# chlhnu/DOT-SOCP

Measured on AMD Instinct MI355X. Metric: ADMM iters/sec on NxNxT dot2d staggered grid at 1/2/4/8 MI355X, higher is better.
Workload: dtype f64

## Files before the change

### dot-socp_amd/csrc/kernels.h

```cpp
#pragma once
#include "common.h"
#include "defer.h"
#include "particle_block.h"

namespace dotsocp {

struct LoopCoef {
    double s;
    double sf;
    double dF;
    double at, ax, ay;
    double tau;
    double c1, c2;
    double dinv1, dinv2;
};

enum {
    S_Q2 = 0, S_Z2, S_APHI2, S_ALPHA2, S_BETA2, S_FBBETA2, S_PRIM1, S_PRIM2, S_DUAL1, S_DUAL2,
    S_COMPLEM, S_DOTCOMP, S_RHO2, S_RHOFQ2, S_MRHOB, S_M2, S_RHOB2, S_QALPHA, S_CPHI, S_PHI2,
    S_COUNT
};

struct KktCoef {
    double sigma;
// ... 134 lines not shown
#define HL_XCHUNK_MAX 32
int launch_hl_pass_y(bool forward, const double *in, double *out, int *arg, i64 n, i64 lines, i64 pitch, hipStream_t st);
int launch_hl_pass_x(bool forward, const double *in, double *out, int *arg, i64 n, i64 lines, i64 pitch, hipStream_t st);
int hl_chunk(int deflt);
int launch_hl_layer(const double *in, double *out, i64 n, double mul, hipStream_t st);
enum { HS_M0 = 0, HS_M1, HS_P0R0, HS_P1R1, HS_HR1, HS_BR0, HS_G1, HS_G0, HS_MAP, HS_COUNT };
enum { HC_G1_MAX = 0, HC_G1_MIN, HC_G0_MAX, HC_G0_MIN, HC_NONFINITE, HC_COUNT };
struct HlReduceArgs {
    i64 ny, nx, py;
    const double *phi0, *phi1, *H, *B, *rho0, *rho1;
    const int *ixf, *iyf, *ixb, *iyb;
    int *arg_fwd, *arg_bwd;
    double hx, hy;
    double *partials;
    unsigned long long *counts;
};
i64 hl_blocks(i64 nodes);
int launch_hl_reduce(const HlReduceArgs &a, double *sums , hipStream_t st);

enum { RR_MAX = 0, RR_MIN, RR_NONFINITE, RR_MASKED, RR_COUNT };
#define RND_LEVELS 255
int launch_rho_range(const Grid &g, const double *alpha, const double *weight, const double *rho0, const double *rho1,
                     const double *a_prev, double sig, double cD, const unsigned char *barrier, unsigned long long *counts,
                     hipStream_t st);
int launch_render(const Grid &g, const double *alpha, const double *weight, const double *rho0, const double *rho1,
                  const double *a_prev, double sig, double cD, i64 tl, int mode, int channels, const unsigned char *barrier,
                  const double *levels, int nlevels, const unsigned char *lut, int barrier_index, double vmax,
                  unsigned char *image, hipStream_t st);
int launch_movement(const Grid &g, const double *alpha, const double *weight, const double *rho0, const double *rho1,
                    const double *a_prev, double sig, double cD, i64 tl, i64 skip_y, i64 skip_x, i64 my, i64 mx, double thr,
                    double *mvX, double *mvY, hipStream_t st);

struct QStepExtra {
    ScaleOps aops;
    double *partials, *resid;
    double kappa, dsD;
    double *u0_tail;
    int c_ends;
};
int launch_qstep_rhs(const Grid &g, const LoopCoef &c, const FusedGeom &fg, const double *phi, const double *q2,
                     const double *sx, const double *sy, const double *weight, const double *tail_bx,
                     const double *tail_by, const double *cvec, double *q_out, const double *alpha_in, double *alpha_out,
                     double *rhs, hipStream_t st, i64 z0 = 0, i64 zcount = -1, i64 zstride = 1,
                     const QStepExtra *ex = nullptr);
i64 qstep_rhs_blocks(const Grid &g, const FusedGeom &fg);
struct QConeArgs {
    const double *phi, *q2v, *sx, *sy, *cvec, *alpha_in, *gamma_in;
    double *alpha_out, *rhs, *q_out, *beta_out, *q2_out, *sx_out, *sy_out;
    i64 TC;
    int ap_on;
    double ap_mul, ap_div;
    int c_ends;
};
int launch_qcone(const Grid &g, const LoopCoef &c, const FusedGeom &fg, QConeArgs a, bool gout, hipStream_t st);
i64 qcone_chunk_len(const Grid &g);
i64 qstep_rhs_chunks(const Grid &g, const FusedGeom &fg, i64 *TC = nullptr);
int launch_qstep_rhs_acc(int var, const Grid &g, const LoopCoef &c, const FusedGeom &fg, const double *phi,
                         const double *q2, const double *sx, const double *sy, const double *weight, const double *cvec,
                         double *q_raw, const double *alpha_in, double *alpha_out, double *rhs, double *q_state,
                         const double *q_anchor, const double *alpha_anchor, const AccCoef &k, hipStream_t st,
                         const double *tail_bx = nullptr, const double *tail_by = nullptr, double *u0_tail = nullptr);
int launch_qstep_palm_first(const Grid &g, const LoopCoef &c, const FusedGeom &fg, const double *phi, const double *q2,
                            const double *sx, const double *sy, const double *cvec, double *q_out, const double *alpha,
                            double *rhs, hipStream_t st, const double *tail_bx = nullptr, const double *tail_by = nullptr,
                            const double *qk = nullptr);

int launch_qstep_fused(const Grid &g, const LoopCoef &c, const FusedGeom &fg, const double *phi,
                       const double *q2, const double *sx, const double *sy, const double *weight,
                       const double *tail_bx, const double *tail_by, double *q_out, double *alpha,
                       hipStream_t st);
int launch_rhs_sigma_fix(const Grid &g, double *rhs, const double *r, double *cvec, double factor, hipStream_t st,
                         bool c_ends = false);
int launch_c_interior_test(const Grid &g, const double *cvec, int *flag, hipStream_t st);
int launch_rhs_fixup(const Grid &g, const LoopCoef &c, const double *u0_prev, double *rhs, hipStream_t st);
int launch_grad(const Grid &g, const LoopCoef &c, const double *phi, double *out, hipStream_t st);
int launch_tail_finalize(const Grid &g, const LoopCoef &c, const FusedGeom &fg, const double *q2, const double *sx,
                         const double *sy, double *tail_bx, double *tail_by, hipStream_t st);
int launch_kkt_tail(const Grid &g, const double *alpha, const double *beta, const double *weight, double *a0,
                    double *a0w, double *bt_bx, double *bt_by, hipStream_t st);
int launch_rhs(const Grid &g, const LoopCoef &c, const double *q, const double *alpha, const double *cvec,
               const double *weight, const double *u0_prev, double *rhs, hipStream_t st, bool c_ends = false);
int launch_qstep(const Grid &g, const LoopCoef &c, const double *phi, const double *z, const double *beta,
                 const double *weight, const double *tail_bx, const double *tail_by, double *q,
                 double *alpha, hipStream_t st);
int launch_u0_tail(const Grid &g, const double *q, const double *alpha, const double *weight, double *out,
                   hipStream_t st);
int launch_scale(double *x, i64 n, double mul, double div, hipStream_t st);
#define DS_MAX_WORLD 64
struct PencilCuts {
    int world;
    i64 cut[DS_MAX_WORLD + 1];
};
int launch_pencil_pack(bool pack, const PencilCuts &pc, i64 plane, i64 ntl, double *slab, double *stage, hipStream_t st);

#define TRI_EXTRA 256
int launch_tri_local(const Grid &g, i64 nt, double kscale, const double *cy, const double *cx, const PencilCuts &pc,
                     const double *r, double *send, hipStream_t st);
int launch_tri_reduced(const Grid &g, i64 nt, double kscale, const double *cy, const double *cx, const PencilCuts &pc,
                       int rank, i64 l0, i64 nl, const i64 *slab_n, const double *recv, double *back, double *zero_work,
                       hipStream_t st, const double *own_recv = nullptr, double *own_back = nullptr);
int launch_tri_final(const Grid &g, i64 nt, double kscale, const double *cy, const double *cx, const PencilCuts &pc,
                     const double *back, double *x, hipStream_t st);
bool tsolve_tri_supported(i64 nt);
bool tsolve_tri_preferred(i64 nt, bool pow2, i64 plane);
bool tsolve_tri_safe(i64 ny, i64 nx, i64 nt);
int launch_tsolve_tri(const Grid &g, i64 nt, double kscale, const double *cy, const double *cx, double *x, hipStream_t st);
int device_cus();
// ... 60 lines not shown
```

### dot-socp_amd/csrc/qstep_march.hip

```cpp
#include "device_utils.h"
#include "gather_tile.h"
#include "kernels.h"
#include "qstep_tile.h"

#include <cstdlib>

namespace dotsocp {


struct QRhsArgs {
    const double *phi, *q2v, *sx, *sy, *weight, *tail_bx, *tail_by, *cvec, *alpha_in;
    double *q_out, *alpha_out, *rhs;
    double *u0_tail;
    i64 TC, z0, zstride;
    double *q_state;
    const double *q_anchor, *alpha_anchor;
    double c1, c2, om_rho, rho;
    APend ap;
    int xcd;
    const double *qk;
    double *partials, *resid;
    double kappa, dsD;
    int c_ends;
};

enum { Q_Q2 = 0, Q_ALPHA2, Q_APHI2, Q_PRIM1, Q_QALPHA, Q_CPHI, Q_PHI2, Q_DUAL1, Q_MRHOB, Q_M2, Q_RHOB2, Q_COUNT };

template <bool WEIGHTED, int VAR, bool KKT = false, int QTX = TILE_X>
__global__ void __launch_bounds__(TILE_Y *QTX, (QTX > TILE_X && !WEIGHTED ? 4 : 1)) k_qstep_rhs(Grid g, LoopCoef c, FusedGeom fg, QRhsArgs a) {
    __shared__ double xch[2][QTX][TILE_Y];
    __shared__ double ph[2][QTX + 2][TILE_Y + 2];
    __shared__ double xcha[KKT ? 2 : 1][KKT ? QTX : 1][KKT ? TILE_Y : 1];
    __shared__ double xchr[KKT ? 2 : 1][KKT ? QTX : 1][KKT ? TILE_Y : 1];
    double S[Q_COUNT];
    if (KKT) {
#pragma unroll
        for (int i = 0; i < Q_COUNT; ++i) S[i] = 0.0;
    }
    auto wgt = [&](i64 k) { return WEIGHTED ? a.weight[k] : 1.0; };
    auto entry = [&](double tmp, double qn, double an, double w) {
        const double wq = w * qn;
        S[Q_Q2] += qn * qn;
        S[Q_ALPHA2] += an * an;
        S[Q_APHI2] += tmp * tmp;
        const double r1 = tmp - wq;
        S[Q_PRIM1] += r1 * r1;
        S[Q_QALPHA] += wq * an;
    };
    double a0prev = 0.0, rhoTprev = 0.0;
    const BlockId blk = block_id(a.xcd != 0);
    const QTile<QTX> t = q_tile<QTX>(g, fg, blk);
    const int lane = t.lane, xl = t.xl;
    const i64 y = t.y, x = t.x;
    const bool inb = t.inb;
    const i64 t0 = ((i64)blk.z * a.zstride + a.z0) * a.TC;
    const i64 t1 = (t0 + a.TC < g.ntl) ? t0 + a.TC : g.ntl;
    auto put = [&](i64 k, double qn, double an, double ain) {
        a.q_out[k] = qn;
// ... 180 lines not shown
    const i64 target = 32768;
    i64 chunks = (target + tiles - 1) / tiles;
    i64 TC = (g.ntl + chunks - 1) / chunks;
    if (TC < 8) TC = 8;
    if (!(g.first && g.last) && cone_split_enabled() && g.ntl >= 12) {
        const i64 tail = (g.ntl / 4 < 4) ? 4 : g.ntl / 4;
        const i64 body = g.ntl - tail, nb = (body + 7) / 8;
        TC = (body + nb - 1) / nb;
    }
    if (TC > g.ntl) TC = g.ntl;
    if (TC < 1) TC = 1;
    if (TCout) *TCout = TC;
    return (g.ntl + TC - 1) / TC;
}

static int launch_qstep_rhs_var(int var, const Grid &g, const LoopCoef &c, const FusedGeom &fg, QRhsArgs a, hipStream_t st,
                                i64 z0, i64 zcount, i64 zstride) {
    i64 TC = 1;
    const i64 chunks = qstep_rhs_chunks(g, fg, &TC);
    if (zcount < 0) zcount = chunks - z0;
    if (z0 < 0 || zcount <= 0 || zstride < 1 || z0 + (zcount - 1) * zstride >= chunks) return 0;
    a.TC = TC;
    a.z0 = z0;
    a.zstride = zstride;
    a.xcd = 1;
    dim3 grid((unsigned)fg.nyblk, (unsigned)fg.nxblk, (unsigned)zcount);
    dim3 blk(TILE_Y, TILE_X);
    const char *qe = getenv("DOTSOCP_QTX");
    const int qtx_env = qe ? atoi(qe) : 0;
    const int qtx = qtx_env ? qtx_env : ((fg.nyblk * fg.nxblk * zcount >= 8192 && !a.weight) ? 2 * TILE_X : TILE_X);
    if (var == 0 && !a.partials && qtx == 2 * TILE_X) {
        dim3 grid2((unsigned)fg.nyblk, (unsigned)((g.nx + 2 * TILE_X - 1) / (2 * TILE_X)), (unsigned)zcount);
        dim3 blk2(TILE_Y, 2 * TILE_X);
        if (a.weight) DS_KLAUNCH((k_qstep_rhs<true, 0, false, 2 * TILE_X>), grid2, blk2, 0, st, g, c, fg, a);
        else DS_KLAUNCH((k_qstep_rhs<false, 0, false, 2 * TILE_X>), grid2, blk2, 0, st, g, c, fg, a);
        DS_HIP(hipGetLastError());
        return 0;
    }
#define QRHS_LAUNCH(W, V) DS_KLAUNCH((k_qstep_rhs<W, V>), grid, blk, 0, st, g, c, fg, a)
    if (var == 0 && a.partials) {
        if (a.weight) DS_KLAUNCH((k_qstep_rhs<true, 0, true>), grid, blk, 0, st, g, c, fg, a);
        else DS_KLAUNCH((k_qstep_rhs<false, 0, true>), grid, blk, 0, st, g, c, fg, a);
    } else if (a.weight) {
        if (var == 0) QRHS_LAUNCH(true, 0); else if (var == 1) QRHS_LAUNCH(true, 1); else QRHS_LAUNCH(true, 2);
    } else {
        if (var == 0) QRHS_LAUNCH(false, 0); else if (var == 1) QRHS_LAUNCH(false, 1);
        else if (var == 2) QRHS_LAUNCH(false, 2); else QRHS_LAUNCH(false, 3);
    }
#undef QRHS_LAUNCH
    DS_HIP(hipGetLastError());
    return 0;
}

template <bool NT, bool GOUT>
__global__ void __launch_bounds__(TILE_Y *TILE_X, 3) k_qcone(Grid g, LoopCoef c, FusedGeom fg, QConeArgs a) {
    constexpr int XB = TILE_X;
    __shared__ double2 xch[2][XB][TILE_Y];
    __shared__ double ph[2][XB + 2][TILE_Y + 2];
    __shared__ double2 gch[2][XB][64];
    const APend ap{a.ap_on, a.ap_mul, a.ap_div};
    const BlockId blk = block_id(true);
    const QTile<XB> t = q_tile<XB>(g, fg, blk);
    const int lane = t.lane, xl = t.xl;
    const i64 y = t.y, x = t.x;
    const bool inb = t.inb;
    const i64 t0 = (i64)blk.z * a.TC;
    const i64 t1 = (t0 + a.TC < g.ntl) ? t0 + a.TC : g.ntl;
    const i64 tstart = (t0 >= 2) ? t0 - 2 : 0;
    const i64 tstop = (t1 == g.ntl) ? t1 + 1 : t1;
    const i64 nxblk = gridDim.y, nyblk = gridDim.x;
    const QSrc src{a.phi, a.q2v, a.sx, a.sy, nullptr, nullptr, nullptr, a.cvec, a.alpha_in, nullptr, a.c_ends};
    double p0 = 0.0;
    if (inb) {
        const i64 node0 = y + g.py * (x + g.nx * tstart);
        p0 = a.phi[node0];
        store_phi_layer<XB>(ph[0], t, p0, load_phi_halo(g, t, a.phi, node0));
    }
    double u0prev = 0.0;
    double q0c = 0.0;
    EdgeQuad eprev{0.0, 0.0, 0.0, 0.0};
    GatherCarry gc;
    int par = 0;
    __syncthreads();
    for (i64 tl = tstart; tl < tstop; ++tl) {
        const bool own = tl >= t0;
        const bool hasC = (tl > tstart) && (tl - 1 < g.ncl);
        const i64 ci = t.yc + g.py * (t.xc + g.nx * (hasC ? tl - 1 : 0));
        double b[10];
        if (hasC) {
#pragma unroll
            for (int j = 0; j < 10; ++j) b[j] = ld_stream<NT>(a.gamma_in + j * g.Nc + ci);
        }
        EdgeQuad ecur{0.0, 0.0, 0.0, 0.0};
        double q0n = 0.0;
        if (tl < g.ntl) {
            const QLayerIn in = q_layer_load<false, XB>(g, c, fg, t, src, ph[par], tl, false, false);
            const QLayerOut o = q_layer_calc<false, 0, XB>(c, t, in, ap, p0, false, false);
            q0n = o.q0n;
            if (own) {
                if (in.hasCell) {
                    a.alpha_out[in.node] = o.a0n;
                    if (!GOUT) a.q_out[in.node] = o.q0n;
                }
                if (t.hasBx) {
                    a.alpha_out[in.eX] = o.aXn;
                    if (!GOUT) a.q_out[in.eX] = o.qXn;
                }
                if (t.hasBy) {
                    a.alpha_out[in.eY] = o.aYn;
                    if (!GOUT) a.q_out[in.eY] = o.qYn;
                }
            }
            xch[par][xl][lane] = make_double2(o.ubx, o.qXn);
            store_phi_layer<XB>(ph[par ^ 1], t, in.pTl, in.h);
            __syncthreads();
            const double uby_s = __shfl_up(o.uby, 1, 64);
            const double qY_s = __shfl_up(o.qYn, 1, 64);
            if (inb) {
                const double2 r = from_left(t, xch[par], make_double2(o.ubx_l, o.qL),
                                            make_double2(0.0, 0.0));
                const double uby_m = from_below(t, uby_s, o.uby_b), qY_m = from_below(t, qY_s, o.qB);
                if (own) a.rhs[in.node] = adjoint_sum(g, c, t, tl, u0prev, o.u0, r.x, o.ubx, uby_m, o.uby) + in.cv;
                ecur.xm = (x >= 1) ? c.sf * r.y : 0.0;
                ecur.xp = (x <= g.nx - 2) ? c.sf * o.qXn : 0.0;
                ecur.ym = (y >= 1) ? c.sf * qY_m : 0.0;
                ecur.yp = (y <= g.ny - 2) ? c.sf * o.qYn : 0.0;
            }
            u0prev = o.u0;
            p0 = o.pT;
            par ^= 1;
        }
        if (tl > tstart) {
            double w[10];
            if (hasC) {
                double v[10];
                build_z2(v, q0c, eprev, ecur, c.s, c.dF);
#pragma unroll
                for (int j = 0; j < 10; ++j) b[j] = mult_finish(b[j], v[j], c.tau);
                if (!GOUT && own && inb) {
#pragma unroll
                    for (int j = 0; j < 10; ++j) st_stream<NT>(a.beta_out + j * g.Nc + ci, b[j]);
                }
#pragma unroll
                for (int j = 0; j < 10; ++j) v[j] = v[j] - b[j];
                proj_row<10>(v);
                if (GOUT && own && inb) {
#pragma unroll
                    for (int j = 0; j < 10; ++j) st_stream<NT>(a.beta_out + j * g.Nc + ci, mult_carry(b[j], v[j], c.tau));
                }
#pragma unroll
                for (int j = 0; j < 10; ++j) w[j] = v[j] + b[j];
                if (own && inb) a.q2_out[ci] = c.s * (w[9] - w[0]);
            } else {
#pragma unroll
                for (int j = 0; j < 10; ++j) w[j] = 0.0;
            }
            gather_emit<XB>(g, c.sf, gch, gc, w, tl - 1, own && inb, x, y, xl, lane, nxblk, nyblk, blk.y, blk.x, a.q2_out,
                            a.sx_out, a.sy_out);
        }
        eprev = ecur;
        q0c = q0n;
    }
}

i64 qcone_chunk_len(const Grid &g) {
    i64 TC = g.ntl;
    if (const char *e = getenv("DOTSOCP_QCONE_TC")) {
        const i64 n = atoll(e);
        if (n >= 1) TC = n;
    }
    return TC < g.ntl ? TC : g.ntl;
}

int launch_qcone(const Grid &g, const LoopCoef &c, const FusedGeom &fg, QConeArgs a, bool gout, hipStream_t st) {
    if (fg.XB != TILE_X || !(g.first && g.last) || g.ncl < 1) { set_error("internal: k_qcone on a grid it does not serve"); return DOTSOCP_ESTATE; }
    a.TC = qcone_chunk_len(g);
    const i64 chunks = (g.ntl + a.TC - 1) / a.TC;
    dim3 grid((unsigned)fg.nyblk, (unsigned)fg.nxblk, (unsigned)chunks);
    dim3 blk(TILE_Y, TILE_X);
    const bool nt = stream_nt_enabled();
    if (gout) {
        if (nt) DS_KLAUNCH((k_qcone<true, true>), grid, blk, 0, st, g, c, fg, a);
        else DS_KLAUNCH((k_qcone<false, true>), grid, blk, 0, st, g, c, fg, a);
    } else {
        if (nt) DS_KLAUNCH((k_qcone<true, false>), grid, blk, 0, st, g, c, fg, a);
        else DS_KLAUNCH((k_qcone<false, false>), grid, blk, 0, st, g, c, fg, a);
    }
    DS_HIP(hipGetLastError());
    return 0;
}

int launch_qstep_palm_first(const Grid &g, const LoopCoef &c, const FusedGeom &fg, const double *phi, const double *q2,
                            const double *sx, const double *sy, const double *cvec, double *q_out, const double *alpha,
                            double *rhs, hipStream_t st, const double *tail_bx, const double *tail_by, const double *qk) {
    QRhsArgs a{};
    a.phi = phi; a.q2v = q2; a.sx = sx; a.sy = sy; a.cvec = cvec; a.tail_bx = tail_bx; a.tail_by = tail_by;
    a.alpha_in = alpha; a.q_out = q_out; a.rhs = rhs; a.qk = qk;
    return launch_qstep_rhs_var(3, g, c, fg, a, st);
}

}
```

### dot-socp_amd/csrc/solver.h

```cpp
#pragma once
#include <chrono>
#include <functional>
#include <memory>
#include <string>
#include <type_traits>
#include <vector>

#include "hostmem.h"
#include "kernels.h"

namespace dotsocp {

constexpr unsigned long long POISON_WORD = 0x7ff8bad0bad0bad0ull;
int guarded_malloc(void **p, size_t bytes, bool fp = false);
void guarded_free(void *p);
bool poison_enabled();
int poison_region(void *p, size_t bytes);
long long device_cache_release();
long long device_cache_held(int dev);
int canary_check(std::string *report);
bool canary_enabled();
bool stream_stress_enabled();
void stream_stress(hipStream_t st);

// ... 37 lines not shown
    }
    int zalloc(double **p, i64 n) {
        DS_CHECK(alloc(p, n));
        DS_HIP(hipMemsetAsync(*p, 0, sizeof(double) * (size_t)(n > 0 ? n : 1), st));
        return 0;
    }
    double *phi = nullptr;
    double *q = nullptr;
    double *alpha = nullptr;
    double *z = nullptr;
    double *beta = nullptr;
    double *c = nullptr;
    bool c_ends = false;
    double *weight = nullptr;
    double *w0 = nullptr, *w1 = nullptr;
    i64 l0 = 0, nl = 0;
    double *pencil = nullptr, *pencil2 = nullptr;
    double *stage = nullptr;
    double *u0_prev = nullptr, *tail_bx = nullptr, *tail_by = nullptr;
    double *a0_prev = nullptr, *a0w_prev = nullptr, *btail_bx = nullptr, *btail_by = nullptr;
    double *send_plane = nullptr, *send_plane2 = nullptr, *send_bx = nullptr, *send_by = nullptr;
    KktWork kw{};
    double *q_old = nullptr, *q2 = nullptr, *beta2 = nullptr, *sx = nullptr, *sy = nullptr;
    double *q3 = nullptr, *p2 = nullptr, *sxp = nullptr, *syp = nullptr;
    double *send_pbx = nullptr, *send_pby = nullptr, *ptail_bx = nullptr, *ptail_by = nullptr;
    double *alpha2 = nullptr;
    double *sx2 = nullptr, *sy2 = nullptr;
    double *tri_send = nullptr, *tri_recv = nullptr, *tri_bsend = nullptr, *tri_brecv = nullptr, *tri_zero = nullptr;
    double *carry = nullptr;
    FusedGeom fg{};
    double *phi_p = nullptr, *alpha_p = nullptr, *z_p = nullptr;
    double *phi_a = nullptr, *q_a = nullptr, *alpha_a = nullptr, *z_a = nullptr, *beta_a = nullptr;
    double *rep_edges = nullptr, *rep_part = nullptr, *rep_sums = nullptr;
    unsigned long long *rep_counts = nullptr;
    double *adv_vel = nullptr;
    i64 adv_have[2] = {-1, -1};
};

#define FOR_SLABS(s) for (auto &s : slabs) if (int rc_use__ = use(s)) return rc_use__; else

int dotsocp_slab_range_impl(i64 nt, int world, int rank, i64 *t0, i64 *t1);
void pencil_range(i64 plane, int world, int j, i64 *l0, i64 *l1);

bool if_adjust_sigma(double iter, double last_iter);

enum Phase { PH_RHS = 0, PH_POISSON, PH_PROJ, PH_QSTEP, PH_BETA, PH_KKT, PH_FUSED_A, PH_FUSED_B, PH_MATERIALISE,
             PH_COMM, PH_INTERP, PH_ACC_CONE, PH_ACC_GATHER, PH_QSTEP0, PH_TRANSPOSE, PH_CONE_CARRY, PH_QCONE, PH_VELOCITY, PH_ADVECT,
             PH_DEPOSIT, PH_FRAME_L1, PH_ADVECT_PATH, PH_MAP_FINAL, PH_HL_PASS_X, PH_HL_PASS_Y, PH_HL_REDUCE, PH_COUNT };

bool rescale_due(i64 it, int rescale, double maxFeas, double relGap);
bool cone_writes_beta(i64 it, double lastSigmaIt, i64 maxit, bool checkStepByStep, bool last_of_run, int rescale,
                      double maxFeas, double relGap);

enum { QCONE_NONE = 0, QCONE_STEADY = 1, QCONE_EXIT = 2 };
int qcone_form(i64 it, double lastSigmaIt, i64 maxit, bool checkStepByStep, bool last_of_run, bool next_last_of_run,
               int rescale, double maxFeas, double relGap);

struct Solver {
    dotsocp_problem prob{};
    int device = 0;
    i64 ny = 0, nx = 0, nt = 0;
    hipStream_t stream = nullptr;
    hipStream_t stream_z = nullptr;
    bool multi_device = false;
    int ndev_visible = 1;
    std::vector<DevRes *> devres;
    int cur_dev = -1;
    std::vector<Slab> slabs;
    std::unique_ptr<DeferCtx> defer;
    int world = 1;
    int rank = 0;
    void *nccl = nullptr;
    double *h_sums = nullptr;
    double *d_red = nullptr;
    bool fused = true;
    bool overlap = false;
    bool tri_tsolve = true;
    bool peer_ok = true;
    bool cross_device = false;
    ~Solver();
    int init(const dotsocp_problem *p, int device, int nslabs, bool multi_dev = false);
    int attach_rccl(const unsigned char *id, int rank, int world);
    int use(const Slab &s);
    int use_dev(int d);
    int sync_all();
    DevRes *res_for(int dev);
    i64 column_pad() const;
    i64 row_pitch() const;
    int alloc_slabs(int first, int count);
    int ensure_alloc();
    void free_slabs();
    bool multi() const { return world > 1; }
    bool remote() const { return nccl != nullptr; }

    int xcopy(Slab &from, const double *src, Slab &to, double *dst, i64 count);
    int xcopy2d(Slab &from, const double *src, size_t spitch, Slab &to, double *dst, size_t dpitch, size_t width,
                size_t height);
    bool comm_z = false;
    bool comm_async = false;
    int comm_depth = 0;
    hipStream_t cst(const Slab &s) const { return comm_z ? s.st_z : s.st; }
    int comm_enter();
    int comm_leave();
    int comm_fork();
    int comm_mark(SlabEvent ev);
    int comm_wait(SlabEvent ev);
    int open_groups = 0;
// ... 33 lines not shown
    int download(int field, double *host);
    int upload_weight_from(const double *src, int src_dev, i64 src_ny, i64 src_nx, i64 src_nt);
    bool c_ends_on = true;
    int detect_c_ends();
    int stage_left_tail();
    int stage_rho_ends(Slab &s, const double *rho0, const double *rho1);
    int canary_after();
    int recover_outputs(const double *rho0, const double *rho1, double *rho, double *Ex, double *Ey, double *q0,
                        double *bx, double *by);
    int jump_from(Solver &coarse);
    int solution_report(const double *rho0, const double *rho1, dotsocp_report *rep, double *layer_mass, double *layer_neg);
    int render_evolution(const double *rho0, const double *rho1, const dotsocp_render_opts *o, const i64 *frame_nodes,
                         const double *levels, const unsigned char *lut, const unsigned char *barrier, unsigned char *image,
                         double *mvX, double *mvY, dotsocp_render_info *info);

    int velocity_stage(const double *rho0, const double *rho1);
    int velocity_layer(Slab &s, i64 tg, double floor);
    int recover_velocity(const double *rho0, const double *rho1, double floor, double *vX, double *vY);
    int advect_particles(const double *rho0, const double *rho1, const dotsocp_advect_opts *o, double *x, double *y,
                         double *traj_x, double *traj_y, i64 *n_clamped);
    int push_mass(const double *rho0, const double *rho1, const dotsocp_push_opts *o, double *x, double *y, const double *mass,
                  const i64 *frame_nodes, double *frames, i64 *n_clamped, double *unit, double *l1);
    int map_report(const double *rho0, const double *rho1, const dotsocp_advect_opts *o, double *x, double *y, const double *mass,
                   dotsocp_map_report_t *rep, double *disp, double *len, double *action);

    int dual_bound(const double *rho0, const double *rho1, dotsocp_dual *res, double *H, double *B, int *arg_fwd, int *arg_bwd);

    bool begun = false, finished = false, stopped = false;
    dotsocp_opts opts{};
    bool checkPrimDualFeas = true;
    double time_limit = 3600.0;
    double sigma = 1.0, sigmaScale = 1.0;
    double cScale = 1.0, dScale = 1.0, D = 1.0, E = 1.0;
    double norm_c = 0.0, norm_d = 0.0;
    double h = 1.0;
    int rescale = 0, use_feasOrg = 0;
    double maxFeas = 0.0, relGap = 0.0, tol_feasOrg = 0.0;
    double lastSigmaIt = 0.0;
    i64 it = 0;
    LoopCoef lc{};
    std::vector<double> hist_kkt, hist_time, hist_iter, hist_gap;
    std::chrono::steady_clock::time_point t_begin;
    double elapsed_prev = 0.0;
    double elapsed_agreed = 0.0;
    bool deferred = false;
    bool z_valid = true;
    bool z_prev_ok = false;
    bool rhs_valid = false;
    bool cone_carry = true;
    bool beta_gamma = false;
    bool cone_gout = false;
    bool last_of_run = false;
    int qcone = -1;
    bool q_valid = true;
    bool early_pass = false;
    bool early_gout = false;
    bool next_last_of_run = false;
    int need_q(const char *who) const;
    int qcone_decide() const;
    bool time_limit_passed() const;
    i64 timeout_at = -1;
    bool timeout_pending = false;
    int need_beta_form(const char *who) const;
    ScaleOps bops{0, 1.0, 1.0, 1.0, 1.0};
    ScaleOps zp_ops{0, 1.0, 1.0, 1.0, 1.0};
    int push_beta_op(double mul, double div);
    int flush_beta();
    ScaleOps aops{0, 1.0, 1.0, 1.0, 1.0};
    int flush_alpha();
    int sigma_scale_folded(double factor);
    FusedArgs pending_step_args(const Slab &s) const;
    double last_S[S_COUNT] = {0};
    double last_S_sigma = 1.0;
    i64 last_S_it = -1;
    bool norm_cache = true;
    bool kkt_fold = true;
    KktCoef kkt_coef() const;
    int clear_partials(Slab &s);
    int begin(const dotsocp_opts *o);
    int begin_method(const dotsocp_opts *o, int method, const dotsocp_acc_opts *acc);
    int run(i64 n_iters, i64 *done);
    int finish(dotsocp_result *res);
    int step(bool *brk);
    int rescale_block();
    int poisson_all(const PhiHooks *hooks = nullptr);
    int poisson_phi();
    int phase_phi(const PhiHooks *hooks = nullptr);
    int phase_z(int part = 0);
    int phase_q(int part = 0, bool kkt = false, int early = QCONE_NONE);
    int phase_mult();
    int materialise();
    int ensure_z();
    int kkt_sums(double *S, bool folded = false);
    int reduce_sums(double *S);
    int norms_light(double *S);
    int kkt_block(bool adjustSigmaYes, bool timed_out, bool *brk, bool folded = false);
    int scale_state(double a_mul, double a_div, double q_div, bool with_c);
    void update_coef();
    double elapsed() const;
    bool profiling = false;
    struct Pending { hipEvent_t a, b; int phase; };
    std::vector<Pending> pending;
    std::vector<hipEvent_t> event_pool;
    double phase_ms[PH_COUNT] = {0};
    i64 phase_launches[PH_COUNT] = {0};
    void prof_begin(int phase, bool on_z = false);
// ... 41 lines not shown
```

### dot-socp_amd/csrc/solver.hip

```cpp
#include "solver.h"

#include <algorithm>
#include <cmath>
#include <cstring>

#include "comm.h"

namespace dotsocp {

void Solver::update_coef() {
    lc.s = E / D;
    lc.sf = edge_factor(lc.s);
    lc.dF = E / dScale;
    const double ht = 1.0 / (double)(nt - 1);
    lc.at = D * (1.0 / ht);
    lc.ax = (nx > 1) ? D * (1.0 / (1.0 / (double)(nx - 1))) : 0.0;
    lc.ay = (ny > 1) ? D * (1.0 / (1.0 / (double)(ny - 1))) : 0.0;
    lc.tau = opts.tau;
    const double tmp = (E / D) * (E / D);
    if (prob.weighted) { lc.c1 = 2.0 * tmp; lc.c2 = tmp; }
    else { lc.c1 = 1.0 + 2.0 * tmp; lc.c2 = 1.0 + tmp; }
    lc.dinv1 = 1.0 / lc.c1;
    lc.dinv2 = 1.0 / lc.c2;
}
// ... 74 lines not shown
    rhs_valid = false;
    if (fused && begun) {
        DS_CHECK(push_beta_op(a_mul, a_div));
    }
    FOR_SLABS(s) {
        const Grid &g = s.g;
        if (with_c) DS_CHECK(launch_scale(s.c, g.Nphi, a_mul, a_div, s.st));
        if (!acc_light) DS_CHECK(launch_scale(s.alpha, g.NqAlloc, a_mul, a_div, s.st));
        if (!(fused && begun) && !acc_light) DS_CHECK(launch_scale(s.beta, 10 * g.Nc, a_mul, a_div, s.st));
        if (q_div != 1.0) {
            DS_CHECK(launch_scale(s.q, g.NqAlloc, 1.0, q_div, s.st));
            if (!(fused && begun) || z_valid) DS_CHECK(launch_scale(s.z, 10 * g.Nc, 1.0, q_div, s.st));
        }
    }
    if (q_div != 1.0 && fused && begun && !z_valid) z_prev_ok = false;
    return 0;
}

int Solver::begin_method(const dotsocp_opts *o, int m, const dotsocp_acc_opts *acc) {
    if (begun) { set_error("begin() called twice"); return DOTSOCP_ESTATE; }
    if (m == DOTSOCP_METHOD_INPALM) return begin(o);
    DS_ARG(m == DOTSOCP_METHOD_ACCADMM || m == DOTSOCP_METHOD_PALM, "unknown method");
    DS_ARG(prob.dim == 2, "the reference has PALM and acc-ADMM loops for 2-D problems only");
    DS_ARG(!(m == DOTSOCP_METHOD_PALM && prob.weighted), "the reference has no weighted PALM loop");
    method = m;
    int rc = begin(o);
    if (rc != 0) { method = DOTSOCP_METHOD_INPALM; return rc; }
    return (m == DOTSOCP_METHOD_PALM) ? palm_begin() : acc_begin(acc);
}

int Solver::begin(const dotsocp_opts *o) {
    DS_ARG(o != nullptr, "opts is NULL");
    DS_ARG(o->maxit >= 0, "opts.maxit < 0");
    DS_ARG(o->sigma > 0, "opts.sigma must be positive");
    if (begun) { set_error("begin() called twice"); return DOTSOCP_ESTATE; }
    cur_dev = -1;
    DS_CHECK(use_dev(device));
    DS_CHECK(ensure_alloc());
    if (method == DOTSOCP_METHOD_ACCADMM) {
        DS_CHECK(acc_alloc());
        fused = false;
    }
    opts = *o;
    cone_carry = true;
    if (const char *e = getenv("DOTSOCP_CONE_CARRY")) cone_carry = (atoi(e) != 0);
    c_ends_on = true;
    if (const char *e = getenv("DOTSOCP_C_ENDS")) c_ends_on = (atoi(e) != 0);
    if (c_ends_on) DS_CHECK(detect_c_ends());
    timeout_at = -1;
    if (const char *e = getenv("DOTSOCP_TEST_TIMEOUT_AT")) timeout_at = atoll(e);
    qcone = -1;
    if (const char *e = getenv("DOTSOCP_QCONE")) qcone = atoi(e);
    if (qcone < -1 || qcone > 2) qcone = -1;
    q_valid = true;
    early_pass = false;
    early_gout = false;
    next_last_of_run = false;
    beta_gamma = false;
    cone_gout = false;
    last_of_run = false;
    timeout_pending = false;
    checkPrimDualFeas = (o->checkPrimDualFeas < 0) ? !prob.weighted : (o->checkPrimDualFeas != 0);
    time_limit = (o->time_limit > 0) ? o->time_limit : 3600.0;
    sigma = o->sigma;
    lastSigmaIt = -INFINITY;
    cScale = prob.cScale; dScale = prob.dScale; D = prob.D; E = prob.E;
    use_feasOrg = 0;
    tol_feasOrg = 5 * o->tol;
    rescale = o->scaling ? 1 : 0;
    maxFeas = INFINITY; relGap = INFINITY;
    h = 1.0 / ((double)nx * (double)ny * (double)nt);
    norm_c = prob.normc; norm_d = prob.normd;
    update_coef();
    DS_CHECK(scale_state(1.0, sigma, 1.0, true));
    DS_CHECK(exchange_q_halo(false));
    sigmaScale = 1.0;
    it = 0;
    stopped = false;
    deferred = false;
    z_valid = true;
    z_prev_ok = false;
    rhs_valid = false;
    last_S_it = -1;
    hist_kkt.clear(); hist_time.clear(); hist_iter.clear(); hist_gap.clear();
    for (int i = 0; i < PH_COUNT; ++i) { phase_ms[i] = 0; phase_launches[i] = 0; }
    if (canary_enabled() && getenv("DOTSOCP_CANARY_SELFTEST")) {
        Slab &s0 = slabs[0];
        DS_CHECK(use(s0));
        const double v = 1.0;
        DS_HIP(ds_memcpy_async(s0.c + s0.g.Nphi, &v, sizeof v, hipMemcpyHostToDevice, s0.st));
        DS_HIP(ds_stream_synchronize(s0.st));
    }
    begun = true;
    elapsed_prev = 0.0;
    elapsed_agreed = 0.0;
    t_begin = std::chrono::steady_clock::now();
    return 0;
}

int Solver::poisson_all(const PhiHooks *hooks) {
    const i64 plane = slabs[0].g.plane;
    const bool tp2 = dct_plan_has_tsolve(devres[0]->pt);
    FOR_SLABS(s) {
        const Grid &g = s.g;
        DS_CHECK(launch_dct_axis(s.res->py, s.w0, s.w1, g.ny, g.nx, g.ntl, 0, 0, s.st, g.py));
        DS_CHECK(launch_dct_axis(s.res->px, s.w1, s.w0, g.ny, g.nx, g.ntl, 1, 0, s.st, g.py));
// ... 102 lines not shown
    }
    const int flavour = (gin ? CONE_GIN : 0) | (gout ? CONE_GOUT : 0);
    const int ph = deferred ? (gin ? PH_CONE_CARRY : PH_FUSED_B) : PH_FUSED_A;
    z_valid = false;
    z_prev_ok = false;
    prof_begin(ph);
    FOR_SLABS(s) {
        FusedArgs a{};
        a.q = s.q;
        a.q2 = s.q2;
        a.sx = s.sx;
        a.sy = s.sy;
        a.beta_in = s.beta;
        a.bops = bops;
        const i64 C = s.fg.chunks;
        const i64 z0 = (part == 2) ? C - 1 : 0;
        const i64 zc = (part == 0) ? C : ((part == 1) ? C - 1 : 1);
        if (deferred) {
            a.q_old = s.q_old;
            a.beta_out = s.beta2;
        }
        const int mode = deferred ? 1 : 0;
        if (s.carry && C > 1) {
            for (i64 z = z0; z < z0 + zc; ++z) {
                a.carry_in = (z > 0) ? s.carry : nullptr;
                a.carry_out = (z + 1 < C) ? s.carry : nullptr;
                DS_CHECK(launch_cone_fused(mode, s.g, lc, s.fg, a, s.st, z, 1, flavour));
            }
        } else {
            DS_CHECK(launch_cone_fused(mode, s.g, lc, s.fg, a, s.st, z0, zc, flavour));
        }
        if (deferred && part != 1) std::swap(s.beta, s.beta2);
    }
    prof_end(ph);
    if (part == 1) return 0;
    if (deferred) {
        bops.clear();
        beta_gamma = gout;
    }
    return 0;
}

KktCoef Solver::kkt_coef() const {
    KktCoef k;
    k.sigma = sigma;
    k.kappa = sigma * cScale * D;
    k.dsD = dScale / D;
    k.dsE = dScale / E;
    return k;
}

int Solver::phase_q(int part, bool kkt, int early) {
    if (!fused) DS_CHECK(flush_alpha());
    if (early != QCONE_NONE && (part != 0 || kkt || multi() || !fused || !deferred || !beta_gamma || !bops.empty())) {
        set_error("internal: early cone pass in a state it does not serve");
        return DOTSOCP_ESTATE;
    }
    const bool egout = (early == QCONE_STEADY);
    const int ph = (early != QCONE_NONE) ? PH_QCONE : PH_QSTEP;
    prof_begin(ph);
    FOR_SLABS(s) {
        hipStream_t st = s.st;
        if (early != QCONE_NONE && qcone != 2) {
            if (!s.sx2) {
                DS_CHECK(s.zalloc(&s.sx2, s.fg.sx_len));
                DS_CHECK(s.zalloc(&s.sy2, s.fg.sy_len));
            }
            QConeArgs a{};
            a.phi = s.phi; a.q2v = s.q2; a.sx = s.sx; a.sy = s.sy; a.cvec = s.c; a.alpha_in = s.alpha; a.gamma_in = s.beta;
            a.alpha_out = s.alpha2; a.rhs = s.w0; a.q_out = s.q_old; a.beta_out = s.beta2;
            a.q2_out = s.q; a.sx_out = s.sx2; a.sy_out = s.sy2;
            a.ap_on = aops.n; a.ap_mul = aops.mul; a.ap_div = aops.div;
            a.c_ends = (c_ends_on && s.c_ends) ? 1 : 0;
            DS_CHECK(launch_qcone(s.g, lc, s.fg, a, egout, st));
            std::swap(s.alpha, s.alpha2);
            std::swap(s.q, s.q_old);
            std::swap(s.q2, s.q_old);
            std::swap(s.sx, s.sx2);
            std::swap(s.sy, s.sy2);
            std::swap(s.beta, s.beta2);
        } else if (!fused) {
            DS_CHECK(launch_qstep(s.g, lc, s.phi, s.z, s.beta, s.weight, s.tail_bx, s.tail_by, s.q, s.alpha, s.st));
        } else {
            const i64 C = qstep_rhs_chunks(s.g, s.fg);
            i64 z0 = 0, zc = C, zs = 1;
            if (part == 1) { zc = C - 1; }
            else if (part == 2) { z0 = C - 1; zc = 1; }
            QStepExtra ex{};
            ex.aops = aops;
            ex.c_ends = (c_ends_on && s.c_ends) ? 1 : 0;
            if (multi() && !s.g.last && part != 1) ex.u0_tail = s.send_plane;
            if (kkt) {
                const KktCoef k = kkt_coef();
                ex.partials = kkt_qstep_partials(s.g, s.kw);
                ex.resid = s.w1;
                ex.kappa = k.kappa; ex.dsD = k.dsD;
            }
            DS_CHECK(launch_qstep_rhs(s.g, lc, s.fg, s.phi, s.q2, s.sx, s.sy, s.weight, s.tail_bx, s.tail_by, s.c,
                                      s.q_old, s.alpha, s.alpha2, s.w0, st, z0, zc, zs, &ex));
            if (part != 1) std::swap(s.alpha, s.alpha2);
            if (part != 1) std::swap(s.q, s.q_old);
            if (early != QCONE_NONE) {
                FusedArgs a{};
                a.q = s.q; a.q2 = s.q2; a.sx = s.sx; a.sy = s.sy;
                a.beta_in = s.beta; a.beta_out = s.beta2;
                a.bops = bops;
                DS_CHECK(launch_cone_fused(1, s.g, lc, s.fg, a, s.st, 0, s.fg.chunks, CONE_GIN | (egout ? CONE_GOUT : 0)));
                std::swap(s.beta, s.beta2);
            }
        }
    }
    prof_end(ph);
    if (part == 1) return 0;
    q_valid = true;
    if (early != QCONE_NONE) {
        q_valid = !egout || qcone == 2;
        beta_gamma = egout;
        z_valid = false;
        z_prev_ok = false;
        early_pass = true;
        early_gout = egout;
    }
    u0_made = multi() && fused;
    if (fused) aops.clear();
    rhs_valid = fused;
    if (multi() && fused && comm_z && cone_split_enabled()) halo_pending = true;
    else DS_CHECK(exchange_q_halo(true));
    return 0;
}

int Solver::phase_mult() {
    if (fused) {
        deferred = true;
        return 0;
    }
    prof_begin(PH_BETA);
    FOR_SLABS(s) DS_CHECK(launch_beta_update(s.g, lc, s.q, s.z, s.beta, s.st));
    prof_end(PH_BETA);
    return 0;
}

int Solver::materialise() {
    if (!fused || !deferred) return 0;
    DS_CHECK(need_beta_form("materialise"));
    DS_CHECK(need_q("materialise"));
    DS_CHECK(ensure_halo());
    prof_begin(PH_MATERIALISE);
    FOR_SLABS(s) {
        FusedArgs a = pending_step_args(s);
        a.beta_out = s.beta;
        a.z_out = s.z;
        DS_CHECK(launch_cone_fused(2, s.g, lc, s.fg, a, s.st));
    }
    prof_end(PH_MATERIALISE);
    bops.clear();
    deferred = false;
    z_valid = true;
    return 0;
}

int Solver::ensure_z() {
    if (!fused || z_valid) return 0;
    DS_CHECK(need_beta_form("ensure_z"));
    DS_CHECK(need_q("ensure_z"));
    if (deferred) return materialise();
    if (!z_prev_ok) {
        set_error("internal: z cannot be regenerated");
        return DOTSOCP_ESTATE;
    }
// ... 143 lines not shown
    if (rescale >= 3 && (it % 100) == 0) {
        DS_CHECK(norms(normPhis, normAlps));
        const double ratio = std::max(normAlps, normPhis) / std::min(normAlps, normPhis);
        if (ratio > 1.2) scaleYes = true;
    }
    const bool first = (rescale == 1) && (maxFeas < 2e-2) && (it >= 10) && (relGap < 5e-2);
    const bool second = (rescale == 2) && (maxFeas < 5e-3) && (it >= 50) && (relGap < 1e-2);
    if (!(first || second || scaleYes)) return 0;
    if (!scaleYes) DS_CHECK(norms(normPhis, normAlps));
    DS_CHECK(materialise());
    const double dScale2 = normPhis, cScale2 = normAlps;
    sigma = sigma * (cScale2 / dScale2);
    norm_c = norm_c / cScale2;
    if (!prob.weighted) norm_d = norm_d / dScale2;
    DS_CHECK(scale_state(dScale2, cScale2 * cScale2, dScale2, true));
    if (method == DOTSOCP_METHOD_PALM) {
        FOR_SLABS(s) DS_CHECK(launch_scale(s.phi, s.g.NphiAlloc, 1.0, dScale2, s.st));
    }
    dScale = dScale2 * dScale;
    cScale = cScale2 * cScale;
    sigmaScale = sigmaScale * (cScale2 / dScale2);
    update_coef();
    rescale += 1;
    return 0;
}

bool rescale_due(i64 it, int rescale, double maxFeas, double relGap) {
    if (rescale >= 3 && (it % 100) == 0) return true;
    if (rescale == 1 && maxFeas < 2e-2 && it >= 10 && relGap < 5e-2) return true;
    if (rescale == 2 && maxFeas < 5e-3 && it >= 50 && relGap < 1e-2) return true;
    return false;
}

bool cone_writes_beta(i64 it, double lastSigmaIt, i64 maxit, bool checkStepByStep, bool last_of_run, int rescale,
                      double maxFeas, double relGap) {
    if (checkStepByStep || if_adjust_sigma((double)it, lastSigmaIt) || it >= maxit) return true;
    if (last_of_run) return true;
    return rescale_due(it + 1, rescale, maxFeas, relGap);
}

int qcone_form(i64 it, double lastSigmaIt, i64 maxit, bool checkStepByStep, bool last_of_run, bool next_last_of_run,
               int rescale, double maxFeas, double relGap) {
    if (cone_writes_beta(it, lastSigmaIt, maxit, checkStepByStep, last_of_run, rescale, maxFeas, relGap)) return QCONE_NONE;
    return cone_writes_beta(it + 1, lastSigmaIt, maxit, checkStepByStep, next_last_of_run, rescale, maxFeas, relGap)
               ? QCONE_EXIT : QCONE_STEADY;
}

bool Solver::time_limit_passed() const {
    return timeout_pending || (remote() ? false : (elapsed() > time_limit || (timeout_at > 0 && it >= timeout_at)));
}

int Solver::qcone_decide() const {
    if (qcone == 0 || !fused || multi() || prob.weighted || method != DOTSOCP_METHOD_INPALM) return QCONE_NONE;
    if (!deferred || !beta_gamma || !bops.empty()) return QCONE_NONE;
    const Slab &s = slabs[0];
    if (s.g.ncl < 1 || s.fg.XB != 4) return QCONE_NONE;
    if (qcone < 0 && s.fg.nyblk * s.fg.nxblk < 2048) return QCONE_NONE;
    if (time_limit_passed()) return QCONE_NONE;
    return qcone_form(it, lastSigmaIt, opts.maxit, opts.ifCheckStepByStep != 0, last_of_run, next_last_of_run, rescale,
                      maxFeas, relGap);
}

bool if_adjust_sigma(double iter, double last_iter) {
    const double passed = iter - last_iter;
    if (iter < 20 && passed >= 3) return true;
    if (iter < 50 && passed >= 6) return true;
    if (iter < 100 && passed >= 10) return true;
    if (iter < 200 && passed >= 15) return true;
    if (iter < 500 && passed >= 25) return true;
    return passed >= 40;
}

static const double kUpdateRule[11][2] = {
    {1.1, 1.10}, {1.2, 1.15}, {1.5, 1.20}, {2, 1.26}, {2.5, 1.28}, {3.33, 1.32},
    {5, 1.35}, {10, 1.40}, {20, 1.60}, {40, 1.80}, {50, 2.00}};

static double get_factor(double xi) {
    double factor = 1.0;
    for (int i = 0; i < 11; ++i) {
        if (xi >= kUpdateRule[i][0]) factor = kUpdateRule[i][1];
        else break;
    }
    return factor;
}

static void adjust_lagrangian_param(double &sigma, double xi, double &factor) {
    factor = 1.0;
    if (xi >= 1) factor = get_factor(xi);
    else if (xi < 1) factor = 1.0 / get_factor(1.0 / xi);
    if (factor != 1.0) {
        const double old = sigma;
        sigma = std::max(std::min(sigma * factor, 1e3), 1e-3);
        factor = sigma / old;
    }
}

int Solver::kkt_block(bool adjustSigmaYes, bool timed_out, bool *brk, bool folded) {
    double S[S_COUNT + 1];
    prof_begin(PH_KKT);
    DS_CHECK(kkt_sums(S, folded));
    prof_end(PH_KKT);
    if (remote()) timed_out = elapsed_agreed > time_limit;
    for (int i = 0; i < S_COUNT; ++i) last_S[i] = S[i];
    last_S_sigma = sigma;
    last_S_it = it;
    const double sh = sqrt(h);
    auto nrm = [&](int i) { return sh * sqrt(S[i]); };
    const double norm_q = nrm(S_Q2), norm_z = nrm(S_Z2), norm_Aphi = nrm(S_APHI2);
    const double norm_alpha = sigma * nrm(S_ALPHA2), norm_beta = sigma * nrm(S_BETA2);
    const double norm_FBbeta = sigma * nrm(S_FBBETA2);
    const double primFea1 = nrm(S_PRIM1), primFea2 = nrm(S_PRIM2);
    const double dualFea1 = sigma * nrm(S_DUAL1), dualFea2 = sigma * nrm(S_DUAL2);
    const double complem = nrm(S_COMPLEM);
// ... 253 lines not shown
```

Measured before the change: 97.05.

## Add entry form of fused q-step/cone kernel for non-deferred iterations

```diff
diff --git a/dot-socp_amd/csrc/kernels.h b/dot-socp_amd/csrc/kernels.h
--- a/dot-socp_amd/csrc/kernels.h
+++ b/dot-socp_amd/csrc/kernels.h
@@ -210,7 +210,16 @@
     double ap_mul, ap_div;
     int c_ends;
 };
-int launch_qcone(const Grid &g, const LoopCoef &c, const FusedGeom &fg, QConeArgs a, bool gout, hipStream_t st);
+struct QConeEntry {
+    const double *qk;
+    ScaleOps bops;
+};
+struct QConeEntryArgs : QConeArgs {
+    const double *qk;
+    ScaleOps bops;
+};
+int launch_qcone(const Grid &g, const LoopCoef &c, const FusedGeom &fg, QConeArgs a, bool gout, hipStream_t st,
+                 const QConeEntry *entry = nullptr);
 i64 qcone_chunk_len(const Grid &g);
 i64 qstep_rhs_chunks(const Grid &g, const FusedGeom &fg, i64 *TC = nullptr);
 int launch_qstep_rhs_acc(int var, const Grid &g, const LoopCoef &c, const FusedGeom &fg, const double *phi,
diff --git a/dot-socp_amd/csrc/qstep_march.hip b/dot-socp_amd/csrc/qstep_march.hip
--- a/dot-socp_amd/csrc/qstep_march.hip
+++ b/dot-socp_amd/csrc/qstep_march.hip
@@ -4,6 +4,7 @@
 #include "qstep_tile.h"
 
 #include <cstdlib>
+#include <type_traits>
 
 namespace dotsocp {
 
@@ -290,12 +291,15 @@
     return 0;
 }
 
-template <bool NT, bool GOUT>
-__global__ void __launch_bounds__(TILE_Y *TILE_X, 3) k_qcone(Grid g, LoopCoef c, FusedGeom fg, QConeArgs a) {
+template <bool NT, bool GOUT, class ARGS = QConeArgs>
+__global__ void __launch_bounds__(TILE_Y *TILE_X, 3) k_qcone(Grid g, LoopCoef c, FusedGeom fg, ARGS a) {
+    constexpr bool GIN = !std::is_same<ARGS, QConeEntryArgs>::value;
+    static_assert(GIN || GOUT, "the entry form always writes gamma");
     constexpr int XB = TILE_X;
     __shared__ double2 xch[2][XB][TILE_Y];
     __shared__ double ph[2][XB + 2][TILE_Y + 2];
     __shared__ double2 gch[2][XB][64];
+    __shared__ double oq[GIN ? 1 : 14][GIN ? 1 : XB][GIN ? 1 : TILE_Y];
     const APend ap{a.ap_on, a.ap_mul, a.ap_div};
     const BlockId blk = block_id(true);
     const QTile<XB> t = q_tile<XB>(g, fg, blk);
@@ -319,19 +323,27 @@
     EdgeQuad eprev{0.0, 0.0, 0.0, 0.0};
     GatherCarry gc;
     int par = 0;
+    if constexpr (!GIN) {
+#pragma unroll
+        for (int k = 9; k < 14; ++k) oq[k][xl][lane] = 0.0;
+    }
     __syncthreads();
     for (i64 tl = tstart; tl < tstop; ++tl) {
         const bool own = tl >= t0;
         const bool hasC = (tl > tstart) && (tl - 1 < g.ncl);
         const i64 ci = t.yc + g.py * (t.xc + g.nx * (hasC ? tl - 1 : 0));
         double b[10];
+        double q0o = 0.0;
         if (hasC) {
 #pragma unroll
             for (int j = 0; j < 10; ++j) b[j] = ld_stream<NT>(a.gamma_in + j * g.Nc + ci);
+            if constexpr (!GIN) q0o = a.qk[ci];
         }
         EdgeQuad ecur{0.0, 0.0, 0.0, 0.0};
         double q0n = 0.0;
         if (tl < g.ntl) {
+            EdgeQuad eo{0.0, 0.0, 0.0, 0.0};
+            if constexpr (!GIN) eo = load_edges(g, a.qk, t.yc, t.xc, tl, c.sf);
             const QLayerIn in = q_layer_load<false, XB>(g, c, fg, t, src, ph[par], tl, false, false);
             const QLayerOut o = q_layer_calc<false, 0, XB>(c, t, in, ap, p0, false, false);
             q0n = o.q0n;
@@ -351,6 +363,20 @@
             }
             xch[par][xl][lane] = make_double2(o.ubx, o.qXn);
             store_phi_layer<XB>(ph[par ^ 1], t, in.pTl, in.h);
+            if constexpr (!GIN) {
+                if (hasC) {
+                    apply_scale_ops(b, a.bops);
+                    const EdgeQuad eop{oq[0][xl][lane], oq[1][xl][lane], oq[2][xl][lane], oq[3][xl][lane]};
+                    double zo[10];
+                    build_z2(zo, q0o, eop, eo, c.s, c.dF);
+#pragma unroll
+                    for (int j = 0; j < 10; ++j) zo[j] = zo[j] - b[j];
+                    proj_row<10>(zo);
+#pragma unroll
+                    for (int j = 0; j < 10; ++j) b[j] = mult_carry(b[j], zo[j], c.tau);
+                }
+                oq[0][xl][lane] = eo.xm; oq[1][xl][lane] = eo.xp; oq[2][xl][lane] = eo.ym; oq[3][xl][lane] = eo.yp;
+            }
             __syncthreads();
             const double uby_s = __shfl_up(o.uby, 1, 64);
             const double qY_s = __shfl_up(o.qYn, 1, 64);
@@ -358,17 +384,24 @@
                 const double2 r = from_left(t, xch[par], make_double2(o.ubx_l, o.qL),
                                             make_double2(0.0, 0.0));
                 const double uby_m = from_below(t, uby_s, o.uby_b), qY_m = from_below(t, qY_s, o.qB);
+                if constexpr (!GIN) u0prev = oq[13][xl][lane];
                 if (own) a.rhs[in.node] = adjoint_sum(g, c, t, tl, u0prev, o.u0, r.x, o.ubx, uby_m, o.uby) + in.cv;
                 ecur.xm = (x >= 1) ? c.sf * r.y : 0.0;
                 ecur.xp = (x <= g.nx - 2) ? c.sf * o.qXn : 0.0;
                 ecur.ym = (y >= 1) ? c.sf * qY_m : 0.0;
                 ecur.yp = (y <= g.ny - 2) ? c.sf * o.qYn : 0.0;
             }
-            u0prev = o.u0;
+            if constexpr (!GIN) oq[13][xl][lane] = o.u0;
+            else u0prev = o.u0;
             p0 = o.pT;
             par ^= 1;
         }
         if (tl > tstart) {
+            if constexpr (!GIN) {
+                eprev = EdgeQuad{oq[4][xl][lane], oq[5][xl][lane], oq[6][xl][lane], oq[7][xl][lane]};
+                q0c = oq[8][xl][lane];
+                gc.p3 = oq[9][xl][lane]; gc.p4 = oq[10][xl][lane]; gc.p7 = oq[11][xl][lane]; gc.p8 = oq[12][xl][lane];
+            }
             double w[10];
             if (hasC) {
                 double v[10];
@@ -395,9 +428,17 @@
             }
             gather_emit<XB>(g, c.sf, gch, gc, w, tl - 1, own && inb, x, y, xl, lane, nxblk, nyblk, blk.y, blk.x, a.q2_out,
                             a.sx_out, a.sy_out);
-        }
-        eprev = ecur;
-        q0c = q0n;
+            if constexpr (!GIN) {
+                oq[9][xl][lane] = gc.p3; oq[10][xl][lane] = gc.p4; oq[11][xl][lane] = gc.p7; oq[12][xl][lane] = gc.p8;
+            }
+        }
+        if constexpr (!GIN) {
+            oq[4][xl][lane] = ecur.xm; oq[5][xl][lane] = ecur.xp; oq[6][xl][lane] = ecur.ym; oq[7][xl][lane] = ecur.yp;
+            oq[8][xl][lane] = q0n;
+        } else {
+            eprev = ecur;
+            q0c = q0n;
+        }
     }
 }
 
@@ -410,14 +451,23 @@
     return TC < g.ntl ? TC : g.ntl;
 }
 
-int launch_qcone(const Grid &g, const LoopCoef &c, const FusedGeom &fg, QConeArgs a, bool gout, hipStream_t st) {
+int launch_qcone(const Grid &g, const LoopCoef &c, const FusedGeom &fg, QConeArgs a, bool gout, hipStream_t st,
+                 const QConeEntry *entry) {
     if (fg.XB != TILE_X || !(g.first && g.last) || g.ncl < 1) { set_error("internal: k_qcone on a grid it does not serve"); return DOTSOCP_ESTATE; }
+    if (entry && (!gout || !entry->qk || a.q2_out == entry->qk)) { set_error("internal: entry form of k_qcone with the wrong buffers"); return DOTSOCP_ESTATE; }
     a.TC = qcone_chunk_len(g);
     const i64 chunks = (g.ntl + a.TC - 1) / a.TC;
     dim3 grid((unsigned)fg.nyblk, (unsigned)fg.nxblk, (unsigned)chunks);
     dim3 blk(TILE_Y, TILE_X);
     const bool nt = stream_nt_enabled();
-    if (gout) {
+    if (entry) {
+        QConeEntryArgs ea{};
+        static_cast<QConeArgs &>(ea) = a;
+        ea.qk = entry->qk;
+        ea.bops = entry->bops;
+        if (nt) DS_KLAUNCH((k_qcone<true, true, QConeEntryArgs>), grid, blk, 0, st, g, c, fg, ea);
+        else DS_KLAUNCH((k_qcone<false, true, QConeEntryArgs>), grid, blk, 0, st, g, c, fg, ea);
+    } else if (gout) {
         if (nt) DS_KLAUNCH((k_qcone<true, true>), grid, blk, 0, st, g, c, fg, a);
         else DS_KLAUNCH((k_qcone<false, true>), grid, blk, 0, st, g, c, fg, a);
     } else {
diff --git a/dot-socp_amd/csrc/solver.h b/dot-socp_amd/csrc/solver.h
--- a/dot-socp_amd/csrc/solver.h
+++ b/dot-socp_amd/csrc/solver.h
@@ -113,7 +113,7 @@
 bool cone_writes_beta(i64 it, double lastSigmaIt, i64 maxit, bool checkStepByStep, bool last_of_run, int rescale,
                       double maxFeas, double relGap);
 
-enum { QCONE_NONE = 0, QCONE_STEADY = 1, QCONE_EXIT = 2 };
+enum { QCONE_NONE = 0, QCONE_STEADY = 1, QCONE_EXIT = 2, QCONE_ENTRY = 3 };
 int qcone_form(i64 it, double lastSigmaIt, i64 maxit, bool checkStepByStep, bool last_of_run, bool next_last_of_run,
                int rescale, double maxFeas, double relGap);
 
@@ -253,6 +253,7 @@
     bool cone_gout = false;
     bool last_of_run = false;
     int qcone = -1;
+    bool qcone_entry = true;
     bool q_valid = true;
     bool early_pass = false;
     bool early_gout = false;
diff --git a/dot-socp_amd/csrc/solver.hip b/dot-socp_amd/csrc/solver.hip
--- a/dot-socp_amd/csrc/solver.hip
+++ b/dot-socp_amd/csrc/solver.hip
@@ -150,6 +150,8 @@
     qcone = -1;
     if (const char *e = getenv("DOTSOCP_QCONE")) qcone = atoi(e);
     if (qcone < -1 || qcone > 2) qcone = -1;
+    qcone_entry = true;
+    if (const char *e = getenv("DOTSOCP_QCONE_ENTRY")) qcone_entry = (atoi(e) != 0);
     q_valid = true;
     early_pass = false;
     early_gout = false;
@@ -358,11 +360,13 @@
 
 int Solver::phase_q(int part, bool kkt, int early) {
     if (!fused) DS_CHECK(flush_alpha());
-    if (early != QCONE_NONE && (part != 0 || kkt || multi() || !fused || !deferred || !beta_gamma || !bops.empty())) {
+    const bool entry = (early == QCONE_ENTRY);
+    if (early != QCONE_NONE && (part != 0 || kkt || multi() || !fused ||
+                                (entry ? (deferred || beta_gamma) : (!deferred || !beta_gamma || !bops.empty())))) {
         set_error("internal: early cone pass in a state it does not serve");
         return DOTSOCP_ESTATE;
     }
-    const bool egout = (early == QCONE_STEADY);
+    const bool egout = (early == QCONE_STEADY) || entry;
     const int ph = (early != QCONE_NONE) ? PH_QCONE : PH_QSTEP;
     prof_begin(ph);
     FOR_SLABS(s) {
@@ -378,9 +382,14 @@
             a.q2_out = s.q; a.sx_out = s.sx2; a.sy_out = s.sy2;
             a.ap_on = aops.n; a.ap_mul = aops.mul; a.ap_div = aops.div;
             a.c_ends = (c_ends_on && s.c_ends) ? 1 : 0;
-            DS_CHECK(launch_qcone(s.g, lc, s.fg, a, egout, st));
+            if (entry) {
+                a.q_out = nullptr;
+                a.q2_out = s.q_old;
+            }
+            const QConeEntry ea{s.q, bops};
+            DS_CHECK(launch_qcone(s.g, lc, s.fg, a, egout, st, entry ? &ea : nullptr));
             std::swap(s.alpha, s.alpha2);
-            std::swap(s.q, s.q_old);
+            if (!entry) std::swap(s.q, s.q_old);
             std::swap(s.q2, s.q_old);
             std::swap(s.sx, s.sx2);
             std::swap(s.sy, s.sy2);
@@ -411,7 +420,9 @@
                 a.q = s.q; a.q2 = s.q2; a.sx = s.sx; a.sy = s.sy;
                 a.beta_in = s.beta; a.beta_out = s.beta2;
                 a.bops = bops;
-                DS_CHECK(launch_cone_fused(1, s.g, lc, s.fg, a, s.st, 0, s.fg.chunks, CONE_GIN | (egout ? CONE_GOUT : 0)));
+                if (entry) a.q_old = s.q_old;
+                DS_CHECK(launch_cone_fused(1, s.g, lc, s.fg, a, s.st, 0, s.fg.chunks,
+                                           (entry ? 0 : CONE_GIN) | (egout ? CONE_GOUT : 0)));
                 std::swap(s.beta, s.beta2);
             }
         }
@@ -421,6 +432,7 @@
     q_valid = true;
     if (early != QCONE_NONE) {
         q_valid = !egout || qcone == 2;
+        bops.clear();
         beta_gamma = egout;
         z_valid = false;
         z_prev_ok = false;
@@ -670,13 +682,16 @@
 
 int Solver::qcone_decide() const {
     if (qcone == 0 || !fused || multi() || prob.weighted || method != DOTSOCP_METHOD_INPALM) return QCONE_NONE;
-    if (!deferred || !beta_gamma || !bops.empty()) return QCONE_NONE;
+    const bool entry = !deferred && !beta_gamma;
+    if (entry ? !(qcone_entry && cone_carry) : (!deferred || !beta_gamma || !bops.empty())) return QCONE_NONE;
     const Slab &s = slabs[0];
     if (s.g.ncl < 1 || s.fg.XB != 4) return QCONE_NONE;
     if (qcone < 0 && s.fg.nyblk * s.fg.nxblk < 2048) return QCONE_NONE;
     if (time_limit_passed()) return QCONE_NONE;
-    return qcone_form(it, lastSigmaIt, opts.maxit, opts.ifCheckStepByStep != 0, last_of_run, next_last_of_run, rescale,
-                      maxFeas, relGap);
+    const int form = qcone_form(it, lastSigmaIt, opts.maxit, opts.ifCheckStepByStep != 0, last_of_run, next_last_of_run, rescale,
+                                maxFeas, relGap);
+    if (entry) return form == QCONE_STEADY ? QCONE_ENTRY : QCONE_NONE;
+    return form;
 }
 
 bool if_adjust_sigma(double iter, double last_iter) {
```

After: 98.17, median of 6. Within noise of the previous version (+1.2%).
